# sizhe-li/neural-jacobian-field

Hardware: AMD Instinct MI355X
Metric: rendered rays/s (64 samples/ray, 256^2 image) (higher is better)
Workload: dtype f32 (v_mfma_f32_32x32x2_f32: exact fp32 products, fp32 accumulate -- the reference's arithmetic)

## Files before the change

### neural-jacobian-field_amd/csrc/njf_device.h

```cpp
#pragma once
#include <hip/hip_runtime.h>
#include <stdint.h>

__device__ __forceinline__ float relu_bits(float x) { return __int_as_float(max(__float_as_int(x), 0)); }

typedef float f32x16 __attribute__((ext_vector_type(16)));
typedef float f32x4 __attribute__((ext_vector_type(4)));
typedef _Float16 f16x8 __attribute__((ext_vector_type(8)));
typedef _Float16 f16x16 __attribute__((ext_vector_type(16)));
typedef _Float16 f16x32 __attribute__((ext_vector_type(32)));
typedef int i32x8 __attribute__((ext_vector_type(8)));
typedef int i32x4 __attribute__((ext_vector_type(4)));
typedef int i32x2 __attribute__((ext_vector_type(2)));
typedef unsigned u32x6 __attribute__((ext_vector_type(6)));

#define PREC_F32 0
#define PREC_F16X2 1
#define PREC_F16F6 2
#define PREC_F16 3

#define NJF_WAVES 4
#define NJF_THREADS (NJF_WAVES * 64)
#define NJF_CHUNK 8192

#define NJF_STREAM_BUFFERS 2
#define LDS_CTR_FLOATS 0
#define LDS_W0 0
#define LDS_W1 NJF_CHUNK
#define LDS_BIAS (NJF_STREAM_BUFFERS * NJF_CHUNK)
#define LDS_BIAS_FLOATS 2752
#define LDS_BIAS_FLOATS_PROPOSAL 1344
#define LDS_SCRATCH_PER_WAVE 528
#define LDS_FLOATS_RENDER (LDS_BIAS + LDS_BIAS_FLOATS + LDS_CTR_FLOATS)
#define LDS_FLOATS_PROPOSAL (LDS_BIAS + LDS_BIAS_FLOATS_PROPOSAL + NJF_WAVES * LDS_SCRATCH_PER_WAVE + LDS_CTR_FLOATS)
#define LDS_SCRATCH_PROPOSAL (LDS_BIAS + LDS_BIAS_FLOATS_PROPOSAL)

extern __shared__ __attribute__((aligned(16))) float njf_lds[];

__device__ __forceinline__ float mfma_step(float a, float b, f32x16& c) {
  c = __builtin_amdgcn_mfma_f32_32x32x2f32(a, b, c, 0, 0, 0);
  return 0.f;
}

#ifdef NJF_STAMPS
#define NJF_STAMP_SLOTS 1024
#ifdef NJF_STAMPS_PROPOSAL
#define NJF_STAMP_BASE LDS_FLOATS_PROPOSAL
#define NJF_STAMP_LOGS_PROPOSAL true
#else
#define NJF_STAMP_BASE LDS_FLOATS_RENDER
#define NJF_STAMP_LOGS_PROPOSAL false
#endif
__device__ unsigned njf_stamp_out[NJF_STAMP_SLOTS];
#define NJF_STAMP_FIELD int stamp_i;
#define NJF_STAMP_INIT(st) (st).stamp_i = -1
#define NJF_STAMP(st, tag)                                                                                   \
  do {                                                                                                       \
    if ((st).stamp_i >= 0 && (st).stamp_i < NJF_STAMP_SLOTS) {                                               \
      njf_lds[NJF_STAMP_BASE + (st).stamp_i] =                                                               \
          __uint_as_float(((unsigned)(tag) << 24) | ((unsigned)__builtin_readcyclecounter() & 0xffffffu));   \
      (st).stamp_i += 1;                                                                                     \
    }                                                                                                        \
  } while (0)
#define NJF_STAMP_P(st, tag) do { if (NJF_STAMP_LOGS_PROPOSAL) NJF_STAMP(st, tag); } while (0)
#define NJF_STAMP_ARM(st, IS_PROPOSAL, wave)                                                                                \
  const bool njf_stamping = ((IS_PROPOSAL) == NJF_STAMP_LOGS_PROPOSAL) && blockIdx.x == gridDim.x / 2 + 3 && (wave) == 1; \
  if (njf_stamping) (st).stamp_i = 0;                                                                                     \
  NJF_STAMP(st, 9)
// ... 125 lines not shown
}
template <bool RELU>
__device__ __forceinline__ void split_pair_u(float x0, float x1, unsigned& hu, unsigned& lu) {
  if (RELU) {
    x0 = relu_bits(x0);
    x1 = relu_bits(x1);
  }
  const f16x2 hp = {(_Float16)x0, (_Float16)x1};
  hu = __builtin_bit_cast(unsigned, hp);
  asm("v_fma_mixlo_f16 %0, -%1, 1.0, %2 op_sel:[0,0,0] op_sel_hi:[1,0,0]" : "=v"(lu) : "v"(hu), "v"(x0));
  asm("v_fma_mixhi_f16 %0, -%1, 1.0, %2 op_sel:[1,0,0] op_sel_hi:[1,0,0]" : "+v"(lu) : "v"(hu), "v"(x1));
}

typedef short s16x2 __attribute__((ext_vector_type(2)));
template <bool RELU>
__device__ __forceinline__ unsigned pack_pair_f16(float x0, float x1) {
  typedef float f32x2 __attribute__((ext_vector_type(2)));
  const f32x2 xp = {x0, x1};
  const f16x2 hp = __builtin_convertvector(xp, f16x2);
  if constexpr (RELU) {
    const s16x2 z = {0, 0};
    return __builtin_bit_cast(unsigned, __builtin_elementwise_max(__builtin_bit_cast(s16x2, hp), z));
  } else {
    return __builtin_bit_cast(unsigned, hp);
  }
}

#define F6_HI 0
#define F6_P1 16384
#define F6_P2 24576
#define F6_SCALE 28672


template <int PREC, int MBO, int NKB, int KB0, bool RELU, int KBI, class ST>
__device__ __forceinline__ void mma_chunk(ST& st, const float* __restrict__ wl, int lane,
                                          const f32x16 (&in)[KBI], f32x16 (&out)[MBO]) {
  constexpr bool SPREAD = MBO == 4 && (NKB == 2 || (PREC == PREC_F16 && NKB == 4)) && NJF_DMA_ROUNDS == 8;
  if constexpr (!SPREAD) stream_flush(st);
  if constexpr (PREC == PREC_F32) {
    const float* base = wl + lane * 4;
#pragma unroll
    for (int kb = 0; kb < NKB; ++kb) {
#pragma unroll
      for (int q = 0; q < 4; ++q) {
        f32x4 a[MBO];
#pragma unroll
        for (int m = 0; m < MBO; ++m) a[m] = *(const f32x4*)(base + ((kb * 4 + q) * MBO + m) * 256);
        if constexpr (SPREAD) {
          if (kb * 4 + q < 4) {
            dma_issue(st, 2 * (kb * 4 + q));
            dma_issue(st, 2 * (kb * 4 + q) + 1);
          }
        }
#pragma unroll
        for (int e = 0; e < 4; ++e) {
          float b = in[KB0 + kb][q * 4 + e];
          if (RELU) b = relu_bits(b);
#pragma unroll
          for (int m = 0; m < MBO; ++m) out[m] = __builtin_amdgcn_mfma_f32_32x32x2f32(a[m][e], b, out[m], 0, 0, 0);
        }
      }
    }
  } else if constexpr (PREC == PREC_F16F6 && MBO == 4 && NKB == 2) {
    typedef __attribute__((address_space(3))) const char* lds_ptr;
    const lds_ptr wb = (lds_ptr)(const char*)wl;
    lds_ptr p16 = wb + lane * 16;
    lds_ptr p8 = wb + lane * 8;
    asm volatile("" : "+v"(p16), "+v"(p8));
    unsigned bh[4][4], bl[4][4], mx[4];
#pragma unroll
    for (int p = 0; p < 4; ++p) {
      split_pair_u<RELU>(in[KB0][2 * p], in[KB0][2 * p + 1], bh[0][p], bl[0][p]);
      mx[p] = RELU ? bh[0][p] : (bh[0][p] & 0x7fff7fffu);
    }
#define NJF_LDS(T) const __attribute__((address_space(3))) T*
    auto hfrag = [&](int i) { return *(NJF_LDS(f16x8))(p16 + i * 1024); };
    auto f6frag = [&](int idx) {
      const i32x4 a4 = *(NJF_LDS(i32x4))(p16 + F6_P1 + idx * 1024);
      const i32x2 b2 = *(volatile NJF_LDS(i32x2))(p8 + F6_P2 + idx * 512);
      return i32x8{a4[0], a4[1], a4[2], a4[3], b2[0], b2[1], 0, 0};
    };
    auto op8 = [](const unsigned (&v)[4]) { return __builtin_bit_cast(f16x8, u32x4{v[0], v[1], v[2], v[3]}); };
// ... 679 lines not shown
    for (int m = 0; m < 4; ++m)
#pragma unroll
      for (int q = 0; q < 2; ++q) {
        u32x4 o;
#pragma unroll
        for (int e = 0; e < 4; ++e) o[e] = pack_pair_f16<DO_RELU>(v[m][8 * q + 2 * e], v[m][8 * q + 2 * e + 1]);
        *(u32x4*)(d16 + 16 * m + 8 * q) = o;
      }
  } else {
#pragma unroll
  for (int m = 0; m < 4; ++m)
#pragma unroll
    for (int q = 0; q < 4; ++q) {
      f32x4 o;
#pragma unroll
      for (int e = 0; e < 4; ++e) o[e] = DO_RELU ? fmaxf(v[m][4 * q + e], 0.f) : v[m][4 * q + e];
      *(f32x4*)(dst + 16 * m + 4 * q) = o;
    }
  }
  if (mask != nullptr) {
    unsigned w[2] = {0u, 0u};
#pragma unroll
    for (int m = 0; m < 4; ++m)
#pragma unroll
      for (int r = 0; r < 16; ++r) {
        const unsigned b = (unsigned)min(max(__float_as_int(v[m][r]), 0), 1);
        w[m >> 1] |= b << (16 * (m & 1) + r);
      }
    typedef unsigned u32x2 __attribute__((ext_vector_type(2)));
    *(u32x2*)mask = u32x2{w[0], w[1]};
  }
}

template <int PREC, bool DUMP = false, int SHARED = 0, class ST>
__device__ __forceinline__ void resnet_tile(ST& st, const float* __restrict__ bias,
                                            const float* __restrict__ gz, const PointGeom& g,
                                            const f32x16 (&pe)[2], int wave, int lane, f32x16 (&out)[1],
                                            ActDump dump = ActDump{nullptr, nullptr, 0}, const TileShareF16* share = nullptr) {
  static_assert(SHARED == 0 || (PREC == PREC_F16 && !DUMP), "the shared tile state exists for the plain-fp16 inference kernels");
  const int hh = lane >> 5;
  constexpr bool FUSED = PREC == PREC_F32 && !DUMP;
  f32x16 h[4], net[4];
#pragma unroll
  for (int m = 0; m < 4; ++m) h[m] = (f32x16)(0.f);
  if (DUMP && dump.pe != nullptr) {
#pragma unroll
    for (int kb = 0; kb < 2; ++kb)
#pragma unroll
      for (int q = 0; q < 4; ++q) {
        f32x4 o;
#pragma unroll
        for (int e = 0; e < 4; ++e) o[e] = pe[kb][4 * q + e];
        *(f32x4*)(dump.pe + 16 * kb + 4 * q) = o;
      }
  }
  {
    const float* wl = stream_step(st, wave, lane);
    if constexpr ((SHARED & 1) != 0) mma_lin_in_f16_packed(st, wl, lane, share->pe, h);
    else if constexpr (FUSED) mma_chunk_gather_f32<0, false, 2>(st, wl, lane, pe, h, gz, g);
    else mma_chunk<PREC, 4, 2, 0, false, 2>(st, wl, lane, pe, h);
  }
  if constexpr (PREC == PREC_F16) {
    static_assert(!DUMP, "the plain-fp16 mode is an inference mode (training forwards dump fp32-class activations)");
    Footprint fp_net;
    if constexpr ((SHARED & 2) != 0) point_footprint(g, fp_net);
    for (int blk = 0; blk < 5; ++blk) {
      if (blk < 3) {
        NJF_STAMP(st, 4);
        if constexpr ((SHARED & 2) != 0) add_hoisted_latent_f16<4>((const _Float16*)map_at<PREC>(gz, blk * 128), g, hh, h, &fp_net);
        else add_hoisted_latent<4, PREC>(map_at<PREC>(gz, blk * 128), g, lane, h);
        NJF_STAMP(st, 5);
      }
      const float* bl = bias + blk * 256;
      bias_init<4, true, PREC>(bl, hh, net);
// ... 13 lines not shown
      NJF_STAMP(st, 4);
      add_hoisted_latent<4, PREC>(gz + blk * 128, g, lane, h);
      NJF_STAMP(st, 5);
    }
    if (DUMP) dump_vec128<true>(dump_layer(dump, 2 * blk), h, dump.mask ? dump.mask + (size_t)(2 * blk) * (dump.stride / 32) : nullptr, dump.half);
    const float* bl = bias + blk * 256;
    bias_init<4, true, PREC>(bl, hh, net);
    {
      {
        const float* wl = stream_step(st, wave, lane);
        mma_chunk<PREC, 4, 2, 0, true, 4>(st, wl, lane, h, net);
      }
      {
        const float* wl = stream_step(st, wave, lane);
        mma_chunk<PREC, 4, 2, 2, true, 4>(st, wl, lane, h, net);
      }
    }
    if (DUMP) dump_vec128<true>(dump_layer(dump, 2 * blk + 1), net, dump.mask ? dump.mask + (size_t)(2 * blk + 1) * (dump.stride / 32) : nullptr, dump.half);
    bias_init<4, false, PREC>(bl + 128, hh, h);
    {
      {
        const float* wl = stream_step(st, wave, lane);
        mma_chunk<PREC, 4, 2, 0, true, 4>(st, wl, lane, net, h);
      }
      {
        const float* wl = stream_step(st, wave, lane);
        bool plain = true;
        if constexpr (FUSED) {
          if (blk < 2) {
            mma_chunk_gather_f32<2, true, 4>(st, wl, lane, net, h, gz + (blk + 1) * 128, g);
            plain = false;
          }
        }
        if (plain) mma_chunk<PREC, 4, 2, 2, true, 4>(st, wl, lane, net, h);
      }
    }
    if (DUMP && dump.feat != nullptr) dump_vec128<false>(dump.feat + (size_t)blk * dump.stride, h);
  }
  if (DUMP) dump_vec128<true>(dump_layer(dump, 10), h, dump.mask ? dump.mask + (size_t)10 * (dump.stride / 32) : nullptr, dump.half);
  bias_init<1, true, PREC>(bias + 1280, hh, out);
  {
    const float* wl = stream_step(st, wave, lane);
    mma_chunk<PREC, 1, 4, 0, true, 4>(st, wl, lane, h, out);
  }
}

struct ColorDump {
  float* in;
  float* act;
  size_t stride;
};

template <bool DO_RELU>
__device__ __forceinline__ void dump_vec32(float* __restrict__ dst, const f32x16 (&v)[2]) {
#pragma unroll
  for (int m = 0; m < 2; ++m)
#pragma unroll
    for (int q = 0; q < 4; ++q) {
      f32x4 o;
#pragma unroll
      for (int e = 0; e < 4; ++e) o[e] = DO_RELU ? fmaxf(v[m][4 * q + e], 0.f) : v[m][4 * q + e];
      *(f32x4*)(dst + 16 * m + 4 * q) = o;
    }
}

template <int PREC, bool DUMP = false, class ST>
__device__ __forceinline__ void color_tile(ST& st, const float* __restrict__ bias, const f32x16 (&cin)[1],
                                           int wave, int lane, f32x16 (&rgb)[1],
                                           ColorDump dump = ColorDump{nullptr, nullptr, 0}) {
  const int hh = lane >> 5;
  const float* wl = stream_step(st, wave, lane);
  f32x16 a[2], b[2];
  a[0] = (f32x16)(0.f);
  a[1] = (f32x16)(0.f);
  mma_chunk<PREC, 2, 1, 0, false, 1>(st, wl, lane, cin, a);
  bias_init<2, true, PREC>(bias, hh, b);
  mma_chunk<PREC, 2, 2, 0, true, 2>(st, wl + 2048, lane, a, b);
  bias_init<1, true, PREC>(bias + 64, hh, rgb);
  mma_chunk<PREC, 1, 2, 0, true, 2>(st, wl + 6144, lane, b, rgb);
  if (DUMP && dump.in != nullptr) {
#pragma unroll
    for (int q = 0; q < 4; ++q) {
      f32x4 o;
#pragma unroll
      for (int e = 0; e < 4; ++e) o[e] = cin[0][4 * q + e];
      *(f32x4*)(dump.in + 4 * q) = o;
    }
    dump_vec32<true>(dump.act, a);
    dump_vec32<true>(dump.act + dump.stride, b);
  }
}

__device__ __forceinline__ float erf_branchless(float a) {
  const float t = fabsf(a), s = a * a;
  float r = fmaf(-1.72853470e-5f, t, 3.83197126e-4f);
  const float u = fmaf(-3.88396438e-3f, t, 2.42546219e-2f);
  r = fmaf(r, s, u);
  r = fmaf(r, t, -1.06777877e-1f);
  r = fmaf(r, t, -6.34846687e-1f);
  r = fmaf(r, t, -1.28717512e-1f);
  r = fmaf(r, t, -t);
  const float hi = copysignf(1.0f - __builtin_amdgcn_exp2f(r * 1.4426950408889634f), a);
  float q = -5.96761703e-4f;
  q = fmaf(q, s, 4.99119423e-3f);
  q = fmaf(q, s, -2.67681349e-2f);
  q = fmaf(q, s, 1.12819925e-1f);
  q = fmaf(q, s, -3.76125336e-1f);
  q = fmaf(q, s, 1.28379166e-1f);
  const float lo = fmaf(q, a, a);
  return t > 0.927734375f ? hi : lo;
}

// ... 198 lines not shown
```

### neural-jacobian-field_amd/csrc/njf_kernels.hip

```cpp
#include <hip/hip_runtime.h>
#include <math.h>
#include <stdint.h>

#include <atomic>
#include <type_traits>

#include "../../include/njf_hip.h"
#include "njf_device.h"

enum {
  NJF_OK = 0,
  NJF_E_NULL = -1,
  NJF_E_SHAPE = -2,
  NJF_E_ACTION_DIM = -3,
  NJF_E_SAMPLES = -4,
  NJF_E_DOUT = -5,
  NJF_E_MODE = -6,
  NJF_E_GMAP = -7,
  NJF_E_VALUE = -8,
};

extern "C" int njf_abi_version(void) { return NJF_ABI_VERSION; }
extern "C" int njf_rays_per_workgroup(void) { return NJF_WAVES; }

// ... 992 lines not shown
  cy /= nrm;
  cz /= nrm;
  const float* m = c2w + b * 16;
  const float dx = fmaf(m[3], 0.0f, fmaf(m[2], cz, fmaf(m[1], cy, m[0] * cx)));
  const float dy = fmaf(m[7], 0.0f, fmaf(m[6], cz, fmaf(m[5], cy, m[4] * cx)));
  const float dz = fmaf(m[11], 0.0f, fmaf(m[10], cz, fmaf(m[9], cy, m[8] * cx)));
  origins[3 * (size_t)i + 0] = m[3];
  origins[3 * (size_t)i + 1] = m[7];
  origins[3 * (size_t)i + 2] = m[11];
  directions[3 * (size_t)i + 0] = dx;
  directions[3 * (size_t)i + 1] = dy;
  directions[3 * (size_t)i + 2] = dz;
  if (z) z[i] = cz;
}

extern "C" int njf_generate_rays(const float* coords, int height, int width, const float* k_inv, const float* c2w,
                                 int batch, int rays, float* origins, float* directions, float* z, void* stream) {
  if (!k_inv || !c2w || !origins || !directions) return NJF_E_NULL;
  if (batch < 1 || rays < 1) return NJF_E_SHAPE;
  if (!coords && (height < 1 || width < 1 || (long long)height * width != rays)) return NJF_E_SHAPE;
  const int n = batch * rays;
  raygen_kernel<<<(n + 255) / 256, 256, 0, (hipStream_t)stream>>>(coords, height, width, k_inv, c2w, batch, rays, origins,
                                                                 directions, z);
  return launch_status();
}

template <int PREC>
constexpr int resnet_chunks() { return PREC == PREC_F16 ? NJF_RESNET_CHUNKS_F16 : NJF_RESNET_CHUNKS; }
template <int PREC>
constexpr int resnet_gap_at() { return PREC == PREC_F16 ? NJF_RESNET_CHUNKS_F16 : 0x7fffffff; }
template <int PREC>
constexpr int resnet_gap() { return PREC == PREC_F16 ? NJF_RESNET_CHUNKS - NJF_RESNET_CHUNKS_F16 : 0; }

struct RayCommon {
  const float* origins;
  const float* directions;
  int rays_per_batch;
  int total_rays;
  NjfCameras cams;
  NjfFeatureMap gmap;
};

__device__ __forceinline__ void load_bias_block(const float* __restrict__ src, int n, int dst_off) {
  for (int i = threadIdx.x; i < n; i += NJF_THREADS) njf_lds[LDS_BIAS + dst_off + i] = src[i];
}

__device__ __forceinline__ float alpha_of(float ds) {
  const float series = ds * fmaf(-0.5f * ds, fmaf(-(1.0f / 3.0f) * ds, fmaf(-0.25f * ds, fmaf(-0.2f, ds, 1.0f), 1.0f), 1.0f), 1.0f);
  return ds < 0.0625f ? series : 1.0f - expf(-ds);
}

__device__ __forceinline__ float tile_weights(float delta, float sigma, bool valid, int j, float& carry) {
  const float ds = (valid && delta > 0.f) ? delta * sigma : 0.f;
  const float incl = half_scan(ds, j);
  float excl = __shfl_up(incl, 1, 32);
  if (j == 0) excl = 0.f;
  excl += carry;
  carry += __shfl(incl, 31, 32);
  return alpha_of(ds) * expf(-excl);
}

__device__ __forceinline__ void pdf_resample_ray(float* __restrict__ sc, const float* __restrict__ bins_in, int s_in,
                                                 const float* __restrict__ u, int s_out, float* __restrict__ bins_out,
                                                 int lane, bool store) {
  float part = 0.f;
  for (int i = lane; i < s_in; i += 64) part += sc[i];
// ... 68 lines not shown
                                              const PointGeom& g, int tex0, int texel_stride) {
  float* act = nullptr;
  if (d.act) act = d.act_f16 ? (float*)((_Float16*)d.act + pidx * 128 + 64 * hh) : d.act + pidx * 128 + 64 * hh;
  ActDump dump{act, d.pe + pidx * 64 + 32 * hh, points * 128, d.mask ? d.mask + pidx * 4 + 2 * hh : nullptr, d.act_f16 != 0};
  if (hh == 0 && d.foot_idx != nullptr) {
    Footprint f;
    point_footprint(g, f);
    int* fi = d.foot_idx + pidx * 4;
    fi[0] = tex0 + f.t00 / texel_stride;
    fi[1] = tex0 + f.t01 / texel_stride;
    fi[2] = tex0 + f.t10 / texel_stride;
    fi[3] = tex0 + f.t11 / texel_stride;
    float* fw = d.foot_w + pidx * 4;
    fw[0] = f.w00;
    fw[1] = f.w01;
    fw[2] = f.w10;
    fw[3] = f.w11;
  }
  return dump;
}

template <int PREC, bool DUMP = false>
__global__ void __launch_bounds__(NJF_THREADS, 2) proposal_kernel(ProposalArgs a) {
  const int tid = threadIdx.x;
  const int wave = __builtin_amdgcn_readfirstlane(tid >> 6);
  const int lane = tid & 63, j = lane & 31, hh = lane >> 5;
  const int wg = xcd_remap(blockIdx.x, gridDim.x);
  const int ray = wg * NJF_WAVES + wave;
  const bool ray_ok = ray < a.rc.total_rays;
  const int rayc = min(ray, a.rc.total_rays - 1);
  const int b = rayc / a.rc.rays_per_batch;

  load_bias_block(a.b_pack, NJF_RESNET_B_FLOATS, 0);
  const int tiles = (a.s_in + 31) >> 5;
  WeightStream st;
  stream_begin(st, a.w_pack, resnet_chunks<PREC>(), tiles, wave, lane);
  NJF_STAMP_ARM(st, true, wave);

  CamCtx cam;
  load_ctx(a.rc.cams.ctxt_w2c, a.rc.cams.ctxt_k, b, cam);
  const float near = a.rc.cams.z_near[b], far = a.rc.cams.z_far[b];
  const float ox = a.rc.origins[3 * (size_t)rayc], oy = a.rc.origins[3 * (size_t)rayc + 1],
              oz = a.rc.origins[3 * (size_t)rayc + 2];
  const float dx = a.rc.directions[3 * (size_t)rayc], dy = a.rc.directions[3 * (size_t)rayc + 1],
              dz = a.rc.directions[3 * (size_t)rayc + 2];
  const float* gz = map_at<PREC>(a.rc.gmap.data, (size_t)b * a.rc.gmap.height * a.rc.gmap.width * a.rc.gmap.stride + a.gmap_offset);
  const float* bins = a.bins_in + (a.bins_per_ray ? (size_t)rayc * (a.s_in + 1) : 0);
  float* sc = njf_lds + LDS_SCRATCH_PROPOSAL + wave * LDS_SCRATCH_PER_WAVE;
  const float* bias = njf_lds + LDS_BIAS;

  float carry = 0.f;
  for (int t = 0; t < tiles; ++t) {
    const int s = t * 32 + j;
    const bool valid = s < a.s_in;
    const int sc_i = min(s, a.s_in - 1);
    const float b0 = bins[sc_i], b1 = bins[sc_i + 1];
    const float start = b0 * far + (1.0f - b0) * near;
    const float end = b1 * far + (1.0f - b1) * near;
    const float se = start + end;
    const float px = ox + (dx * se) / 2.0f, py = oy + (dy * se) / 2.0f, pz = oz + (dz * se) / 2.0f;
    PointGeom g;
    point_geometry(cam, px, py, pz, a.rc.gmap.height, a.rc.gmap.width, a.rc.gmap.stride, 0u, g);
    NJF_STAMP_P(st, 10);
    f32x16 pe[2];
    positional_encoding(g.xc, g.yc, g.zc, hh, pe);
    f32x16 out[1];
    ActDump dump{nullptr, nullptr, 0};
    if (DUMP && valid && ray_ok)
      dump = point_dump(a.dump, (size_t)ray * a.s_in + s, (size_t)a.rc.total_rays * a.s_in, hh, g,
                        b * a.rc.gmap.height * a.rc.gmap.width, a.rc.gmap.stride);
    resnet_tile<PREC, DUMP>(st, bias, gz, g, pe, wave, lane, out, dump);
    NJF_STAMP_P(st, 14);
    const float pre = __shfl(out[0][0], j, 64);
    const float sigma = expf(pre - 1.0f);
    const float w = tile_weights(end - start, sigma, valid, j, carry);
    if (valid && hh == 0) {
      float wa = w;
      if (a.anneal != 1.0f) wa = powf(w, a.anneal);
      sc[s] = wa + 0.01f;
      if (ray_ok) {
        if (a.weights_out) a.weights_out[(size_t)ray * a.s_in + s] = w;
        if (a.density_out) a.density_out[(size_t)ray * a.s_in + s] = sigma;
      }
    }
  }
  NJF_STAMP_P(st, 13);
  __syncthreads();
  const float* u = a.u + (a.u_per_ray ? (size_t)rayc * (a.s_out + 1) : 0);
  pdf_resample_ray(sc, bins, a.s_in, u, a.s_out, a.bins_out + (size_t)rayc * (a.s_out + 1), lane, ray_ok);
  NJF_STAMP_FLUSH(st, 15, lane);
}

template <int PREC, int DUMP, int SHARE = 0, class ST>
__device__ __forceinline__ float density_stage(ST& st, const float* __restrict__ gz_d, const PointGeom& g, int wave,
                                               int lane, f32x16 (&geo)[1], ActDump dump, TileShareF16* share = nullptr) {
  const int j = lane & 31, hh = lane >> 5;
  f32x16 pe[2];
  positional_encoding(g.xc, g.yc, g.zc, hh, pe);
  if constexpr (SHARE != 0) {
    share_tile(pe, *share);
    resnet_tile<PREC, false, SHARE>(st, njf_lds + LDS_BIAS, gz_d, g, pe, wave, lane, geo, dump, share);
  } else {
    resnet_tile<PREC, DUMP == 2>(st, njf_lds + LDS_BIAS, gz_d, g, pe, wave, lane, geo, dump);
  }
  return expf(__shfl(geo[0][15], j, 64) - 1.0f);
}

template <int PREC, int DUMP, class ST>
__device__ __forceinline__ void color_stage(ST& st, const f32x16 (&geo)[1], float dirx, float diry, float dirz,
                                            int wave, int lane, float (&rgb)[3], ColorDump cdump) {
  const int j = lane & 31, hh = lane >> 5;
  asm volatile("" : "+v"(dirx), "+v"(diry), "+v"(dirz));
  float sh[16];
  sh4(dirx, diry, dirz, sh);
  f32x16 cin[1], crgb[1];
#pragma unroll
  for (int r = 0; r < 16; ++r) cin[0][r] = hh ? sh[r] : (r < 15 ? geo[0][r] : 1.0f);
  color_tile<PREC, DUMP == 2>(st, njf_lds + LDS_BIAS + NJF_RESNET_B_FLOATS, cin, wave, lane, crgb, cdump);
#pragma unroll
  for (int c = 0; c < 3; ++c) {
    const float x = __shfl(crgb[0][c], j, 64);
    rgb[c] = 1.0f / (1.0f + expf(-x));
  }
}

template <int JKIND, int PREC, int DUMP, int SHARE = 0, class ST>
__device__ __forceinline__ void jacobian_stage(ST& st, const float* __restrict__ gz_j, const PointGeom& g,
                                               const float* __restrict__ action, int action_dim, int wave, int lane,
                                               f32x16 (&jac)[1], float (&flow)[3], ActDump dump, const TileShareF16* share = nullptr) {
  const int hh = lane >> 5;
  const float* bias = njf_lds + LDS_BIAS + NJF_RESNET_B_FLOATS + NJF_COLOR_B_FLOATS;
  if constexpr (SHARE != 0) {
    static_assert(JKIND == 1 && DUMP == 0, "shared tile state: ResnetFC Jacobian head, inference");
    NJF_STAMP(st, 6);
    NJF_STAMP(st, 7);
    f32x16 unused[2];
    resnet_tile<PREC, false, SHARE>(st, bias, gz_j, g, unused, wave, lane, jac, dump, share);
  } else {
  float xc = g.xc, yc = g.yc, zc = g.zc;
  asm volatile("" : "+v"(xc), "+v"(yc), "+v"(zc) : : "memory");
  f32x16 pe[2];
  NJF_STAMP(st, 6);
  positional_encoding(xc, yc, zc, hh, pe);
  NJF_STAMP_PIN("+v"(pe[0]), "+v"(pe[1]));
  NJF_STAMP(st, 7);
  if (JKIND == 1)
    resnet_tile<PREC, DUMP == 1>(st, bias, gz_j, g, pe, wave, lane, jac, dump);
  else {
    if (DUMP == 1 && dump.pe != nullptr) {
#pragma unroll
      for (int kb = 0; kb < 2; ++kb)
#pragma unroll
        for (int q = 0; q < 4; ++q) {
          f32x4 o;
#pragma unroll
          for (int e = 0; e < 4; ++e) o[e] = pe[kb][4 * q + e];
// ... 35 lines not shown
struct SamplePlace {
  float delta, tm, px, py, pz;
};
__device__ __forceinline__ void place_sample(float b0, float b1, float near, float far, float ox,
                                             float oy, float oz, float dx, float dy, float dz, SamplePlace& sp) {
  asm volatile("" : "+v"(b0), "+v"(b1));
  const float start = b0 * far + (1.0f - b0) * near;
  const float end = b1 * far + (1.0f - b1) * near;
  const float se = start + end;
  sp.delta = end - start;
  sp.tm = se / 2.0f;
  sp.px = ox + (dx * se) / 2.0f;
  sp.py = oy + (dy * se) / 2.0f;
  sp.pz = oz + (dz * se) / 2.0f;
}

template <int JKIND, int PREC, int DUMP = 0, bool AF = true, int PRECJ = PREC>
__global__ void __launch_bounds__(NJF_THREADS, 2) render_kernel(RenderArgs a) {
  constexpr bool WITH_J = JKIND != 0;
  constexpr int J_CHUNKS = JKIND == 1 ? resnet_chunks<PRECJ>() : (JKIND == 2 ? NJF_TRANSFORMER_CHUNKS : 0);
  constexpr int J_BIAS = JKIND == 1 ? NJF_RESNET_B_FLOATS : NJF_TRANSFORMER_B_FLOATS;
  const int tid = threadIdx.x;
  const int wave = __builtin_amdgcn_readfirstlane(tid >> 6);
  const int lane = tid & 63, j = lane & 31, hh = lane >> 5;
  const int wg = xcd_remap(blockIdx.x, gridDim.x);
  const int ray = wg * NJF_WAVES + wave;
  const bool ray_ok = ray < a.rc.total_rays;
  const int rayc = min(ray, a.rc.total_rays - 1);
  const int b = rayc / a.rc.rays_per_batch;
  const int S = a.samples;

  load_bias_block(a.b_d, NJF_RESNET_B_FLOATS, 0);
  load_bias_block(a.b_c, NJF_COLOR_B_FLOATS, NJF_RESNET_B_FLOATS);
  if (WITH_J) load_bias_block(a.b_j, J_BIAS, NJF_RESNET_B_FLOATS + NJF_COLOR_B_FLOATS);
  const int tiles = (S + 31) >> 5;
  WeightStreamT<resnet_gap_at<PREC>(), resnet_gap<PREC>()> st;
  stream_begin(st, a.w_all, resnet_chunks<PREC>() + 1 + J_CHUNKS, tiles, wave, lane);
  NJF_STAMP_ARM(st, false, wave);

  CamCtx cam;
  load_ctx(a.rc.cams.ctxt_w2c, a.rc.cams.ctxt_k, b, cam);
  const float near = a.rc.cams.z_near[b], far = a.rc.cams.z_far[b];
  const float ox = a.rc.origins[3 * (size_t)rayc], oy = a.rc.origins[3 * (size_t)rayc + 1],
              oz = a.rc.origins[3 * (size_t)rayc + 2];
  const float dx = a.rc.directions[3 * (size_t)rayc], dy = a.rc.directions[3 * (size_t)rayc + 1],
              dz = a.rc.directions[3 * (size_t)rayc + 2];
  const size_t gbase = (size_t)b * a.rc.gmap.height * a.rc.gmap.width * a.rc.gmap.stride;
  const float* gz_d = map_at<PREC>(a.rc.gmap.data, gbase + a.goff_d);
  const float* gz_j = map_at<PRECJ>(a.rc.gmap.data, gbase + a.goff_j);
  const float* bins = a.bins + (size_t)rayc * (S + 1);
  const int A = a.rc.cams.action_dim;
  const float* action = a.rc.cams.action ? a.rc.cams.action + (size_t)b * A : nullptr;

  float carry = 0.f;
  float acc_rgb[3] = {0.f, 0.f, 0.f}, acc_w = 0.f, acc_wt = 0.f;
  float acc_p[3] = {0.f, 0.f, 0.f}, acc_pw[3] = {0.f, 0.f, 0.f};
  float tmin = 3.0e38f, tmax = -3.0e38f;
  f32x16 acc_j = (f32x16)(0.f);
  const bool want_af = AF && WITH_J && a.out.action_features != nullptr;

  for (int t = 0; t < tiles; ++t) {
    const int s = t * 32 + j;
    const bool valid = s < S;
    const int sc_i = min(s, S - 1);
    const size_t si = (size_t)ray * S + s;
    const bool store = valid && ray_ok;
// ... 301 lines not shown
  const float* xyz;
  const float* dirs;
  int points_per_batch;
  int total_points;
  NjfCameras cams;
  NjfFeatureMap gmap;
  int goff_d, goff_j;
  const float* w_all;
  const float* b_d;
  const float* b_c;
  const float* b_j;
  float* density;
  float* color;
  float* flow;
  float* jacobian;
  float* geo;
  float* features;
};

template <int MODE, int PREC, int PRECJ = PREC, bool FEAT = false>
__global__ void __launch_bounds__(NJF_THREADS, 2) points_kernel(PointsArgs a) {
  const int tid = threadIdx.x;
  const int wave = __builtin_amdgcn_readfirstlane(tid >> 6);
  const int lane = tid & 63, j = lane & 31, hh = lane >> 5;
  const int wg = xcd_remap(blockIdx.x, gridDim.x);
  const int tile = wg * NJF_WAVES + wave;
  const int p = tile * 32 + j;
  const bool ok = p < a.total_points;
  const int pc = min(p, a.total_points - 1);
  const int b = pc / a.points_per_batch;

  load_bias_block(a.b_d, NJF_RESNET_B_FLOATS, 0);
  if (MODE >= 1) load_bias_block(a.b_c, NJF_COLOR_B_FLOATS, NJF_RESNET_B_FLOATS);
  if (MODE == 2) load_bias_block(a.b_j, NJF_RESNET_B_FLOATS, NJF_RESNET_B_FLOATS + NJF_COLOR_B_FLOATS);
  if (MODE == 3) load_bias_block(a.b_j, NJF_TRANSFORMER_B_FLOATS, NJF_RESNET_B_FLOATS + NJF_COLOR_B_FLOATS);
  WeightStreamT<resnet_gap_at<PREC>(), resnet_gap<PREC>()> st;
  stream_begin(st, a.w_all,
               MODE == 0 ? resnet_chunks<PREC>()
                         : resnet_chunks<PREC>() + 1 + (MODE == 2 ? resnet_chunks<PRECJ>() : (MODE == 3 ? NJF_TRANSFORMER_CHUNKS : 0)),
               1, wave, lane);
  CamCtx cam;
  load_ctx(a.cams.ctxt_w2c, a.cams.ctxt_k, b, cam);
  const float px = a.xyz[3 * (size_t)pc], py = a.xyz[3 * (size_t)pc + 1], pz = a.xyz[3 * (size_t)pc + 2];
  PointGeom g;
  const unsigned gbase = (unsigned)b * (unsigned)(a.gmap.height * a.gmap.width) * (unsigned)a.gmap.stride;
  point_geometry(cam, px, py, pz, a.gmap.height, a.gmap.width, a.gmap.stride, gbase, g);
  const float* bias = njf_lds + LDS_BIAS;
  if (MODE == 0) {
    f32x16 pe[2], out[1];
    positional_encoding(g.xc, g.yc, g.zc, hh, pe);
    resnet_tile<PREC>(st, bias, map_at<PREC>(a.gmap.data, a.goff_d), g, pe, wave, lane, out);
    if (ok && hh == 0 && a.density) a.density[p] = expf(out[0][0] - 1.0f);
  } else {
    float dx = 0.f, dy = 0.f, dz = 1.f;
    if (a.dirs) {
      dx = a.dirs[3 * (size_t)pc];
      dy = a.dirs[3 * (size_t)pc + 1];
      dz = a.dirs[3 * (size_t)pc + 2];
    }
    const int A = a.cams.action_dim;
    const float* action = a.cams.action ? a.cams.action + (size_t)b * A : nullptr;
    constexpr int JK = MODE >= 2 ? MODE - 1 : 0;
    const ActDump nodump{nullptr, nullptr, 0};
    f32x16 geo[1];
    const float sigma = density_stage<PREC, 0>(st, map_at<PREC>(a.gmap.data, a.goff_d), g, wave, lane, geo, nodump);
    if (ok && hh == 0) {
      if (a.density) a.density[p] = sigma;
      if (a.geo) {
#pragma unroll
        for (int r = 0; r < 15; ++r) a.geo[15 * (size_t)p + r] = geo[0][r];
      }
    }
    {
      float rgb[3];
      color_stage<PREC, 0>(st, geo, dx, dy, dz, wave, lane, rgb, ColorDump{nullptr, nullptr, 0});
      if (ok && hh == 0 && a.color) {
        a.color[3 * (size_t)p] = rgb[0];
        a.color[3 * (size_t)p + 1] = rgb[1];
        a.color[3 * (size_t)p + 2] = rgb[2];
      }
    }
    if (JK != 0) {
      f32x16 jac[1];
      float flow[3];
// ... 51 lines not shown
  pz = fmaf((float)iz, l.grid.step[2], l.grid.origin[2]);
}

struct FieldArgs {
  FieldList list;
  float dirx, diry, dirz;
  NjfCameras cams;
  NjfFeatureMap gmap;
  int goff_d, goff_j;
  const float* w_all;
  const float* b_d;
  const float* b_c;
  const float* b_j;
  float* density;
  float* color;
  float* jacobian;
};

template <int MODE, int PREC, int PRECJ = PREC>
__global__ void __launch_bounds__(NJF_THREADS, 2) field_points_kernel(FieldArgs a) {
  const int entries = field_entries(a.list);
  const int tid = threadIdx.x;
  const int wave = __builtin_amdgcn_readfirstlane(tid >> 6);
  const int lane = tid & 63, j = lane & 31, hh = lane >> 5;
  const int wg = xcd_remap(blockIdx.x, gridDim.x);
  if (wg * (NJF_WAVES * 32) >= entries) return;
  const int tile = wg * NJF_WAVES + wave;
  const int p = tile * 32 + j;
  const bool ok = p < entries;
  const int pc = min(p, entries - 1);

  load_bias_block(a.b_d, NJF_RESNET_B_FLOATS, 0);
  if (MODE >= 2) load_bias_block(a.b_c, NJF_COLOR_B_FLOATS, NJF_RESNET_B_FLOATS);
  if (MODE == 3) load_bias_block(a.b_j, NJF_RESNET_B_FLOATS, NJF_RESNET_B_FLOATS + NJF_COLOR_B_FLOATS);
  if (MODE == 4) load_bias_block(a.b_j, NJF_TRANSFORMER_B_FLOATS, NJF_RESNET_B_FLOATS + NJF_COLOR_B_FLOATS);
  WeightStreamT<resnet_gap_at<PREC>(), resnet_gap<PREC>()> st;
  stream_begin(st, a.w_all,
               MODE <= 1 ? resnet_chunks<PREC>()
                         : resnet_chunks<PREC>() + 1 + (MODE == 3 ? resnet_chunks<PRECJ>() : (MODE == 4 ? NJF_TRANSFORMER_CHUNKS : 0)),
               1, wave, lane);
  int b;
  float px, py, pz;
  field_node(a.list, field_global_index(a.list, pc), b, px, py, pz);
  CamCtx cam;
  load_ctx(a.cams.ctxt_w2c, a.cams.ctxt_k, b, cam);
  PointGeom g;
  const unsigned gbase = (unsigned)b * (unsigned)(a.gmap.height * a.gmap.width) * (unsigned)a.gmap.stride;
  point_geometry(cam, px, py, pz, a.gmap.height, a.gmap.width, a.gmap.stride, gbase, g);
  const float* bias = njf_lds + LDS_BIAS;
  if (MODE == 0) {
    f32x16 pe[2], out[1];
    positional_encoding(g.xc, g.yc, g.zc, hh, pe);
    resnet_tile<PREC>(st, bias, map_at<PREC>(a.gmap.data, a.goff_d), g, pe, wave, lane, out);
    if (ok && hh == 0) a.density[p] = expf(out[0][0] - 1.0f);
  } else {
    const int A = a.cams.action_dim;
    constexpr int JK = MODE >= 3 ? MODE - 2 : 0;
    const ActDump nodump{nullptr, nullptr, 0};
    f32x16 geo[1];
    const float sigma = density_stage<PREC, 0>(st, map_at<PREC>(a.gmap.data, a.goff_d), g, wave, lane, geo, nodump);
    if (ok && hh == 0 && a.density) a.density[p] = sigma;
    if (MODE >= 2) {
      float rgb[3];
      color_stage<PREC, 0>(st, geo, a.dirx, a.diry, a.dirz, wave, lane, rgb, ColorDump{nullptr, nullptr, 0});
      if (ok && hh == 0 && a.color) {
        a.color[3 * (size_t)p] = rgb[0];
        a.color[3 * (size_t)p + 1] = rgb[1];
        a.color[3 * (size_t)p + 2] = rgb[2];
      }
    }
    if (JK != 0) {
      f32x16 jac[1];
      float flow[3];
      jacobian_stage<JK, PRECJ, 0>(st, map_at<PRECJ>(a.gmap.data, a.goff_j), g, nullptr, A, wave, lane, jac, flow, nodump);
      if (ok && a.jacobian) {
#pragma unroll
        for (int r = 0; r < 16; ++r) {
          const int d = 16 * hh + r;
          if (d < 3 * A) a.jacobian[(size_t)p * (3 * A) + d] = jac[0][r];
        }
      }
    }
  }
}

__global__ void __launch_bounds__(256) field_xyz_kernel(FieldList l, float* __restrict__ xyz) {
// ... 389 lines not shown
  const int* node;
  const int* count;
  int capacity;
  int nodes, total;
  float dirx, diry, dirz;
  NjfCameras cams;
  NjfFeatureMap gmap;
  int goff_d, goff_j;
  const float* w_all;
  const float* b_d;
  const float* b_c;
  const float* b_j;
  float* density;
  float* color;
  float* jacobian;
};

template <int MODE, int PREC, int PRECJ = PREC>
__global__ void __launch_bounds__(NJF_THREADS, 2) field_at_kernel(FieldAtArgs a) {
  static_assert(MODE >= 2 && MODE <= 4, "decoder modes with the colour head");
  const int entries = a.count ? min(max(*a.count, 0), a.capacity) : a.capacity;
  const int tid = threadIdx.x;
  const int wave = __builtin_amdgcn_readfirstlane(tid >> 6);
  const int lane = tid & 63, j = lane & 31, hh = lane >> 5;
  const int wg = xcd_remap(blockIdx.x, gridDim.x);
  if (wg * (NJF_WAVES * 32) >= entries) return;
  const int tile = wg * NJF_WAVES + wave;
  const int p = tile * 32 + j;
  const bool ok = p < entries;
  const int pc = min(p, entries - 1);

  load_bias_block(a.b_d, NJF_RESNET_B_FLOATS, 0);
  load_bias_block(a.b_c, NJF_COLOR_B_FLOATS, NJF_RESNET_B_FLOATS);
  if (MODE == 3) load_bias_block(a.b_j, NJF_RESNET_B_FLOATS, NJF_RESNET_B_FLOATS + NJF_COLOR_B_FLOATS);
  if (MODE == 4) load_bias_block(a.b_j, NJF_TRANSFORMER_B_FLOATS, NJF_RESNET_B_FLOATS + NJF_COLOR_B_FLOATS);
  WeightStreamT<resnet_gap_at<PREC>(), resnet_gap<PREC>()> st;
  stream_begin(st, a.w_all,
               resnet_chunks<PREC>() + 1 + (MODE == 3 ? resnet_chunks<PRECJ>() : (MODE == 4 ? NJF_TRANSFORMER_CHUNKS : 0)), 1, wave,
               lane);
  const int b = min(max(a.node[pc], 0), a.total - 1) / a.nodes;
  const float px = a.xyz[3 * (size_t)pc], py = a.xyz[3 * (size_t)pc + 1], pz = a.xyz[3 * (size_t)pc + 2];
  CamCtx cam;
  load_ctx(a.cams.ctxt_w2c, a.cams.ctxt_k, b, cam);
  PointGeom g;
  const unsigned gbase = (unsigned)b * (unsigned)(a.gmap.height * a.gmap.width) * (unsigned)a.gmap.stride;
  point_geometry(cam, px, py, pz, a.gmap.height, a.gmap.width, a.gmap.stride, gbase, g);
  const int A = a.cams.action_dim;
  constexpr int JK = MODE >= 3 ? MODE - 2 : 0;
  const ActDump nodump{nullptr, nullptr, 0};
  f32x16 geo[1];
  const float sigma = density_stage<PREC, 0>(st, map_at<PREC>(a.gmap.data, a.goff_d), g, wave, lane, geo, nodump);
  if (ok && hh == 0 && a.density) a.density[p] = sigma;
  {
    float rgb[3];
    color_stage<PREC, 0>(st, geo, a.dirx, a.diry, a.dirz, wave, lane, rgb, ColorDump{nullptr, nullptr, 0});
    if (ok && hh == 0 && a.color) {
      a.color[3 * (size_t)p] = rgb[0];
      a.color[3 * (size_t)p + 1] = rgb[1];
      a.color[3 * (size_t)p + 2] = rgb[2];
    }
  }
  if (JK != 0) {
    f32x16 jac[1];
    float flow[3];
    jacobian_stage<JK, PRECJ, 0>(st, map_at<PRECJ>(a.gmap.data, a.goff_j), g, nullptr, A, wave, lane, jac, flow, nodump);
    if (ok && a.jacobian) {
// ... 2526 lines not shown
```

Measured before the change: 2.017 million.

## Compute narrow output layers on VALU from LDS-resident rows instead of MFMA

The 1-row density output of the fp32 proposal ResNet and the 3-row RGB output of the colour head were computed with full 32x32 MFMA tiles, most of whose rows are wasted. They are now computed as per-lane FMA dot products against the few needed weight rows, which are preloaded into enlarged LDS bias space, with a cross-half shuffle to finish the reduction. The proposal network streams one fewer weight chunk, and the DMA prefetch is skipped when the penultimate chunk is last. This cuts MFMA issue and weight streaming for the output layers, at the cost of a little more LDS per workgroup and extra VALU work.

```diff
diff --git a/neural-jacobian-field_amd/csrc/njf_device.h b/neural-jacobian-field_amd/csrc/njf_device.h
--- a/neural-jacobian-field_amd/csrc/njf_device.h
+++ b/neural-jacobian-field_amd/csrc/njf_device.h
@@ -28,12 +28,16 @@
 #define LDS_W0 0
 #define LDS_W1 NJF_CHUNK
 #define LDS_BIAS (NJF_STREAM_BUFFERS * NJF_CHUNK)
-#define LDS_BIAS_FLOATS 2752
-#define LDS_BIAS_FLOATS_PROPOSAL 1344
+#define LDS_BIAS_FLOATS 2944
+#define LDS_BIAS_FLOATS_PROPOSAL 1472
+#define LDS_BIAS_WOUT1 1344
+#define LDS_BIAS_WRGB 2752
 #define LDS_SCRATCH_PER_WAVE 528
 #define LDS_FLOATS_RENDER (LDS_BIAS + LDS_BIAS_FLOATS + LDS_CTR_FLOATS)
 #define LDS_FLOATS_PROPOSAL (LDS_BIAS + LDS_BIAS_FLOATS_PROPOSAL + NJF_WAVES * LDS_SCRATCH_PER_WAVE + LDS_CTR_FLOATS)
 #define LDS_SCRATCH_PROPOSAL (LDS_BIAS + LDS_BIAS_FLOATS_PROPOSAL)
+static_assert(2 * 4 * LDS_FLOATS_RENDER <= 160 * 1024 && 2 * 4 * LDS_FLOATS_PROPOSAL <= 160 * 1024,
+              "two workgroups per CU (render 77,312 B, proposal 79,872 B each)");
 
 extern __shared__ __attribute__((aligned(16))) float njf_lds[];
 
@@ -225,13 +229,15 @@
 #define F6_SCALE 28672
 
 
-template <int PREC, int MBO, int NKB, int KB0, bool RELU, int KBI, class ST>
+template <int PREC, int MBO, int NKB, int KB0, bool RELU, int KBI, bool MAY_BE_LAST = false, class ST>
 __device__ __forceinline__ void mma_chunk(ST& st, const float* __restrict__ wl, int lane,
                                           const f32x16 (&in)[KBI], f32x16 (&out)[MBO]) {
+  static_assert(!MAY_BE_LAST || PREC == PREC_F32, "only the exact-fp32 proposal network ends on an interleaving chunk");
   constexpr bool SPREAD = MBO == 4 && (NKB == 2 || (PREC == PREC_F16 && NKB == 4)) && NJF_DMA_ROUNDS == 8;
   if constexpr (!SPREAD) stream_flush(st);
   if constexpr (PREC == PREC_F32) {
     const float* base = wl + lane * 4;
+    const bool pending = !MAY_BE_LAST || st.dma_next == 0;
 #pragma unroll
     for (int kb = 0; kb < NKB; ++kb) {
 #pragma unroll
@@ -240,7 +246,7 @@
 #pragma unroll
         for (int m = 0; m < MBO; ++m) a[m] = *(const f32x4*)(base + ((kb * 4 + q) * MBO + m) * 256);
         if constexpr (SPREAD) {
-          if (kb * 4 + q < 4) {
+          if (kb * 4 + q < 4 && pending) {
             dma_issue(st, 2 * (kb * 4 + q));
             dma_issue(st, 2 * (kb * 4 + q) + 1);
           }
@@ -986,7 +992,47 @@
   }
 }
 
-template <int PREC, bool DUMP = false, int SHARED = 0, class ST>
+template <int ROWS, int KBI>
+__device__ __forceinline__ void narrow_out_valu(const float* __restrict__ w, const float* __restrict__ bias, int hh,
+                                                const f32x16 (&in)[KBI], float (&out)[ROWS]) {
+  static_assert(KBI == 2 || KBI == 4, "pairwise combination of the per-block chains");
+  const float* wh = w + 16 * KBI * hh;
+  float acc[ROWS][KBI];
+#pragma unroll
+  for (int c = 0; c < ROWS; ++c)
+#pragma unroll
+    for (int m = 0; m < KBI; ++m) acc[c][m] = 0.f;
+#pragma unroll
+  for (int m = 0; m < KBI; ++m)
+#pragma unroll
+    for (int q = 0; q < 4; ++q)
+#pragma unroll
+      for (int c = 0; c < ROWS; ++c) {
+        const f32x4 v = *(const f32x4*)(wh + c * (32 * KBI) + 16 * m + 4 * q);
+#pragma unroll
+        for (int e = 0; e < 4; ++e) acc[c][m] = fmaf(v[e], relu_bits(in[m][4 * q + e]), acc[c][m]);
+      }
+#pragma unroll
+  for (int c = 0; c < ROWS; ++c) {
+    float s = acc[c][0] + acc[c][1];
+    if constexpr (KBI == 4) s += acc[c][2] + acc[c][3];
+    s += __shfl_xor(s, 32, 64);
+    out[c] = s + bias[c];
+  }
+}
+
+template <int ROWS, int KB>
+__device__ __forceinline__ void load_narrow_rows(const float* __restrict__ packed, float* __restrict__ dst) {
+  static_assert(ROWS <= 4, "rows 0-3 of a block are lanes 0-3");
+  constexpr int K = 32 * KB;
+  for (int i = threadIdx.x; i < ROWS * K; i += NJF_THREADS) {
+    const int f = i / K, k = i % K;
+    const int kh = k / (16 * KB), kk = k % (16 * KB);
+    dst[i] = packed[((kk >> 2) * 64 + 32 * kh + f) * 4 + (kk & 3)];
+  }
+}
+
+template <int PREC, bool DUMP = false, int SHARED = 0, bool OUT1 = false, class ST>
 __device__ __forceinline__ void resnet_tile(ST& st, const float* __restrict__ bias,
                                             const float* __restrict__ gz, const PointGeom& g,
                                             const f32x16 (&pe)[2], int wave, int lane, f32x16 (&out)[1],
@@ -994,6 +1040,7 @@
   static_assert(SHARED == 0 || (PREC == PREC_F16 && !DUMP), "the shared tile state exists for the plain-fp16 inference kernels");
   const int hh = lane >> 5;
   constexpr bool FUSED = PREC == PREC_F32 && !DUMP;
+  constexpr bool OUT_VALU = PREC == PREC_F32 && OUT1;
   f32x16 h[4], net[4];
 #pragma unroll
   for (int m = 0; m < 4; ++m) h[m] = (f32x16)(0.f);
@@ -1073,14 +1120,18 @@
             plain = false;
           }
         }
-        if (plain) mma_chunk<PREC, 4, 2, 2, true, 4>(st, wl, lane, net, h);
+        if (plain) mma_chunk<PREC, 4, 2, 2, true, 4, OUT_VALU>(st, wl, lane, net, h);
       }
     }
     if (DUMP && dump.feat != nullptr) dump_vec128<false>(dump.feat + (size_t)blk * dump.stride, h);
   }
   if (DUMP) dump_vec128<true>(dump_layer(dump, 10), h, dump.mask ? dump.mask + (size_t)10 * (dump.stride / 32) : nullptr, dump.half);
-  bias_init<1, true, PREC>(bias + 1280, hh, out);
-  {
+  if constexpr (OUT_VALU) {
+    float pre[1];
+    narrow_out_valu<1, 4>(bias + LDS_BIAS_WOUT1, bias + 1280, hh, h, pre);
+    out[0][0] = pre[0];
+  } else {
+    bias_init<1, true, PREC>(bias + 1280, hh, out);
     const float* wl = stream_step(st, wave, lane);
     mma_chunk<PREC, 1, 4, 0, true, 4>(st, wl, lane, h, out);
   }
@@ -1107,7 +1158,7 @@
 
 template <int PREC, bool DUMP = false, class ST>
 __device__ __forceinline__ void color_tile(ST& st, const float* __restrict__ bias, const f32x16 (&cin)[1],
-                                           int wave, int lane, f32x16 (&rgb)[1],
+                                           int wave, int lane, float (&rgb)[3],
                                            ColorDump dump = ColorDump{nullptr, nullptr, 0}) {
   const int hh = lane >> 5;
   const float* wl = stream_step(st, wave, lane);
@@ -1117,8 +1168,15 @@
   mma_chunk<PREC, 2, 1, 0, false, 1>(st, wl, lane, cin, a);
   bias_init<2, true, PREC>(bias, hh, b);
   mma_chunk<PREC, 2, 2, 0, true, 2>(st, wl + 2048, lane, a, b);
-  bias_init<1, true, PREC>(bias + 64, hh, rgb);
-  mma_chunk<PREC, 1, 2, 0, true, 2>(st, wl + 6144, lane, b, rgb);
+  if constexpr (PREC == PREC_F32) {
+    narrow_out_valu<3, 2>(njf_lds + LDS_BIAS + LDS_BIAS_WRGB, bias + 64, hh, b, rgb);
+  } else {
+    f32x16 o[1];
+    bias_init<1, true, PREC>(bias + 64, hh, o);
+    mma_chunk<PREC, 1, 2, 0, true, 2>(st, wl + 6144, lane, b, o);
+#pragma unroll
+    for (int c = 0; c < 3; ++c) rgb[c] = __shfl(o[0][c], lane & 31, 64);
+  }
   if (DUMP && dump.in != nullptr) {
 #pragma unroll
     for (int q = 0; q < 4; ++q) {
diff --git a/neural-jacobian-field_amd/csrc/njf_kernels.hip b/neural-jacobian-field_amd/csrc/njf_kernels.hip
--- a/neural-jacobian-field_amd/csrc/njf_kernels.hip
+++ b/neural-jacobian-field_amd/csrc/njf_kernels.hip
@@ -1048,6 +1048,19 @@
 template <int PREC>
 constexpr int resnet_gap() { return PREC == PREC_F16 ? NJF_RESNET_CHUNKS - NJF_RESNET_CHUNKS_F16 : 0; }
 
+template <int PREC>
+constexpr int proposal_chunks() { return PREC == PREC_F32 ? NJF_RESNET_CHUNKS - 1 : resnet_chunks<PREC>(); }
+template <int PREC>
+__device__ __forceinline__ void load_proposal_row(const float* __restrict__ w_pack) {
+  if constexpr (PREC == PREC_F32)
+    load_narrow_rows<1, 4>(w_pack + (NJF_RESNET_CHUNKS - 1) * NJF_CHUNK, njf_lds + LDS_BIAS + LDS_BIAS_WOUT1);
+}
+template <int PREC>
+__device__ __forceinline__ void load_color_rows(const float* __restrict__ w_all) {
+  if constexpr (PREC == PREC_F32)
+    load_narrow_rows<3, 2>(w_all + NJF_RESNET_CHUNKS * NJF_CHUNK + 6144, njf_lds + LDS_BIAS + LDS_BIAS_WRGB);
+}
+
 struct RayCommon {
   const float* origins;
   const float* directions;
@@ -1182,9 +1195,10 @@
   const int b = rayc / a.rc.rays_per_batch;
 
   load_bias_block(a.b_pack, NJF_RESNET_B_FLOATS, 0);
+  load_proposal_row<PREC>(a.w_pack);
   const int tiles = (a.s_in + 31) >> 5;
   WeightStream st;
-  stream_begin(st, a.w_pack, resnet_chunks<PREC>(), tiles, wave, lane);
+  stream_begin(st, a.w_pack, proposal_chunks<PREC>(), tiles, wave, lane);
   NJF_STAMP_ARM(st, true, wave);
 
   CamCtx cam;
@@ -1219,7 +1233,7 @@
     if (DUMP && valid && ray_ok)
       dump = point_dump(a.dump, (size_t)ray * a.s_in + s, (size_t)a.rc.total_rays * a.s_in, hh, g,
                         b * a.rc.gmap.height * a.rc.gmap.width, a.rc.gmap.stride);
-    resnet_tile<PREC, DUMP>(st, bias, gz, g, pe, wave, lane, out, dump);
+    resnet_tile<PREC, DUMP, 0, true>(st, bias, gz, g, pe, wave, lane, out, dump);
     NJF_STAMP_P(st, 14);
     const float pre = __shfl(out[0][0], j, 64);
     const float sigma = expf(pre - 1.0f);
@@ -1263,15 +1277,13 @@
   asm volatile("" : "+v"(dirx), "+v"(diry), "+v"(dirz));
   float sh[16];
   sh4(dirx, diry, dirz, sh);
-  f32x16 cin[1], crgb[1];
+  f32x16 cin[1];
+  float crgb[3];
 #pragma unroll
   for (int r = 0; r < 16; ++r) cin[0][r] = hh ? sh[r] : (r < 15 ? geo[0][r] : 1.0f);
   color_tile<PREC, DUMP == 2>(st, njf_lds + LDS_BIAS + NJF_RESNET_B_FLOATS, cin, wave, lane, crgb, cdump);
 #pragma unroll
-  for (int c = 0; c < 3; ++c) {
-    const float x = __shfl(crgb[0][c], j, 64);
-    rgb[c] = 1.0f / (1.0f + expf(-x));
-  }
+  for (int c = 0; c < 3; ++c) rgb[c] = 1.0f / (1.0f + expf(-crgb[c]));
 }
 
 template <int JKIND, int PREC, int DUMP, int SHARE = 0, class ST>
@@ -1373,6 +1385,7 @@
 
   load_bias_block(a.b_d, NJF_RESNET_B_FLOATS, 0);
   load_bias_block(a.b_c, NJF_COLOR_B_FLOATS, NJF_RESNET_B_FLOATS);
+  load_color_rows<PREC>(a.w_all);
   if (WITH_J) load_bias_block(a.b_j, J_BIAS, NJF_RESNET_B_FLOATS + NJF_COLOR_B_FLOATS);
   const int tiles = (S + 31) >> 5;
   WeightStreamT<resnet_gap_at<PREC>(), resnet_gap<PREC>()> st;
@@ -1740,11 +1753,13 @@
 
   load_bias_block(a.b_d, NJF_RESNET_B_FLOATS, 0);
   if (MODE >= 1) load_bias_block(a.b_c, NJF_COLOR_B_FLOATS, NJF_RESNET_B_FLOATS);
+  if (MODE >= 1) load_color_rows<PREC>(a.w_all);
+  else load_proposal_row<PREC>(a.w_all);
   if (MODE == 2) load_bias_block(a.b_j, NJF_RESNET_B_FLOATS, NJF_RESNET_B_FLOATS + NJF_COLOR_B_FLOATS);
   if (MODE == 3) load_bias_block(a.b_j, NJF_TRANSFORMER_B_FLOATS, NJF_RESNET_B_FLOATS + NJF_COLOR_B_FLOATS);
   WeightStreamT<resnet_gap_at<PREC>(), resnet_gap<PREC>()> st;
   stream_begin(st, a.w_all,
-               MODE == 0 ? resnet_chunks<PREC>()
+               MODE == 0 ? proposal_chunks<PREC>()
                          : resnet_chunks<PREC>() + 1 + (MODE == 2 ? resnet_chunks<PRECJ>() : (MODE == 3 ? NJF_TRANSFORMER_CHUNKS : 0)),
                1, wave, lane);
   CamCtx cam;
@@ -1757,7 +1772,7 @@
   if (MODE == 0) {
     f32x16 pe[2], out[1];
     positional_encoding(g.xc, g.yc, g.zc, hh, pe);
-    resnet_tile<PREC>(st, bias, map_at<PREC>(a.gmap.data, a.goff_d), g, pe, wave, lane, out);
+    resnet_tile<PREC, false, 0, true>(st, bias, map_at<PREC>(a.gmap.data, a.goff_d), g, pe, wave, lane, out);
     if (ok && hh == 0 && a.density) a.density[p] = expf(out[0][0] - 1.0f);
   } else {
     float dx = 0.f, dy = 0.f, dz = 1.f;
@@ -1875,11 +1890,13 @@
 
   load_bias_block(a.b_d, NJF_RESNET_B_FLOATS, 0);
   if (MODE >= 2) load_bias_block(a.b_c, NJF_COLOR_B_FLOATS, NJF_RESNET_B_FLOATS);
+  if (MODE >= 2) load_color_rows<PREC>(a.w_all);
+  if (MODE == 0) load_proposal_row<PREC>(a.w_all);
   if (MODE == 3) load_bias_block(a.b_j, NJF_RESNET_B_FLOATS, NJF_RESNET_B_FLOATS + NJF_COLOR_B_FLOATS);
   if (MODE == 4) load_bias_block(a.b_j, NJF_TRANSFORMER_B_FLOATS, NJF_RESNET_B_FLOATS + NJF_COLOR_B_FLOATS);
   WeightStreamT<resnet_gap_at<PREC>(), resnet_gap<PREC>()> st;
   stream_begin(st, a.w_all,
-               MODE <= 1 ? resnet_chunks<PREC>()
+               MODE == 0 ? proposal_chunks<PREC>() : MODE == 1 ? resnet_chunks<PREC>()
                          : resnet_chunks<PREC>() + 1 + (MODE == 3 ? resnet_chunks<PRECJ>() : (MODE == 4 ? NJF_TRANSFORMER_CHUNKS : 0)),
                1, wave, lane);
   int b;
@@ -1894,7 +1911,7 @@
   if (MODE == 0) {
     f32x16 pe[2], out[1];
     positional_encoding(g.xc, g.yc, g.zc, hh, pe);
-    resnet_tile<PREC>(st, bias, map_at<PREC>(a.gmap.data, a.goff_d), g, pe, wave, lane, out);
+    resnet_tile<PREC, false, 0, true>(st, bias, map_at<PREC>(a.gmap.data, a.goff_d), g, pe, wave, lane, out);
     if (ok && hh == 0) a.density[p] = expf(out[0][0] - 1.0f);
   } else {
     const int A = a.cams.action_dim;
@@ -2350,6 +2367,7 @@
 
   load_bias_block(a.b_d, NJF_RESNET_B_FLOATS, 0);
   load_bias_block(a.b_c, NJF_COLOR_B_FLOATS, NJF_RESNET_B_FLOATS);
+  load_color_rows<PREC>(a.w_all);
   if (MODE == 3) load_bias_block(a.b_j, NJF_RESNET_B_FLOATS, NJF_RESNET_B_FLOATS + NJF_COLOR_B_FLOATS);
   if (MODE == 4) load_bias_block(a.b_j, NJF_TRANSFORMER_B_FLOATS, NJF_RESNET_B_FLOATS + NJF_COLOR_B_FLOATS);
   WeightStreamT<resnet_gap_at<PREC>(), resnet_gap<PREC>()> st;
```

Result: no change. 2.033 million, median of 6 (+0.8%).
